# megaease/easevoice-trainer

Measured on AMD Instinct MI355X. Metric: audio-seconds/sec trained (s2), higher is better.
Workload: dtype bf16; 1 GPU; s2 SoVITS generator+discriminator GAN step, batch=16/GPU, 4 s 32 kHz clips (T=200 frames), configs/s2.json, random-init weights; global_batch=16, parallelism=dp1, launch=hip-graph replay (3 graphs/step)

## Files before the change

easevoice_trainer_amd/csrc/elementwise.hip:

```cpp
#include "evt_common.h"
#include "../../include/evt.h"

namespace {

__device__ __forceinline__ void store_w(void* base, long idx, float w, int dtype) {
  if (dtype == EVT_DT_HALF) reinterpret_cast<h16_t*>(base)[idx] = f2h(w);
  else reinterpret_cast<float*>(base)[idx] = w;
}

__device__ __forceinline__ long reg_idx(const evt_wlayout& L, int d0, int d1, int kk) {
  const int chunk = d1 / L.reg_ck, cc = d1 - chunk * L.reg_ck;
  return (((long)d0 * L.reg_nchunk + chunk) * L.reg_kp + kk) * L.reg_ck + cc;
}

__device__ __forceinline__ long alt_idx(const evt_wlayout& L, int d0, int d1, int kk) {
  const int chunk = d0 / L.alt_ck, cc = d0 - chunk * L.alt_ck;
  if (L.stride == 1) {
    const int t = L.k - 1 - kk;
    return (((long)d1 * L.alt_nchunk + chunk) * L.alt_kp + t) * L.alt_ck + cc;
  }
  const int J = (L.k + L.stride - 1) / L.stride;
  const int ph = kk % L.stride, j = kk / L.stride;
  const int jp = J - 1 - j;
  return ((((long)ph * L.d1 + d1) * L.alt_nchunk + chunk) * L.alt_kp + jp) * L.alt_ck + cc;
// ... 483 lines not shown
  if (found) {
    *scale = *scale * backoff;
    *tracker = 0;
  } else {
    const int ok = *tracker + 1;
    if (ok == interval) {
      const float ns = *scale * growth;
      if (isfinite(ns)) *scale = ns;
      *tracker = 0;
    } else {
      *tracker = ok;
    }
  }
}

__global__ __launch_bounds__(256) void sumsq_kernel(const float* x, long n, float* out) {
  __shared__ float red[4];
  float acc = 0.f;
  for (long i = blockIdx.x * 256L + threadIdx.x; i < n; i += (long)gridDim.x * 256) acc += x[i] * x[i];
  acc = block_reduce_sum_256(acc, red);
  if (threadIdx.x == 0) atomicAdd(out, acc);
}

inline int grid_for(long n, int cap = 8192) {
  long b = (n + 255) / 256;
  if (b > cap) b = cap;
  if (b < 1) b = 1;
  return (int)b;
}

}

#include <stdarg.h>
#include <stdio.h>
static bool g_tags_on = false;
static thread_local char g_last_tag[128] = "";
extern "C" void evt_set_last_tag(const char* fmt, ...) {
  if (!g_tags_on) return;
  va_list ap;
  va_start(ap, fmt);
  vsnprintf(g_last_tag, sizeof(g_last_tag), fmt, ap);
  va_end(ap);
}

extern "C" {

// ... 3 lines not shown
#ifndef EVT_SRC_HASH
#define EVT_SRC_HASH "unknown"
#endif
const char* evt_version(void) { return "evt-hip 0.3 (gfx950, half = " EVT_HALF_NAME ") src=" EVT_SRC_HASH; }
int32_t evt_half_dtype(void) { return EVT_DT_HALF; }

int evt_wn_fold_multi(const evt_wprep_item* items, const int32_t* row_index, int32_t nrows, void* stream) {
  if (!items || !row_index || nrows <= 0) return EVT_EINVAL;
  const int nblocks = ((nrows + 255) / 256) * 256;
  hipLaunchKernelGGL(wn_fold_kernel, dim3(nblocks), dim3(256), 0, (hipStream_t)stream, items, row_index, nrows);
  return evt_check_launch();
}

int evt_wn_fold_groups(const evt_wprep_item* items, const int32_t* group_index, int32_t ngroups, void* stream) {
  if (!items || !group_index || ngroups <= 0) return EVT_EINVAL;
  const int nblocks = ((ngroups + 31) / 32) * 32;
  hipLaunchKernelGGL(wn_fold8_kernel, dim3(nblocks), dim3(256), 0, (hipStream_t)stream, items, group_index, ngroups);
  return evt_check_launch();
}

int evt_wn_grad_multi(const evt_wprep_item* items, const int32_t* row_index, int32_t nrows, void* stream) {
  if (!items || !row_index || nrows <= 0) return EVT_EINVAL;
  hipLaunchKernelGGL(wn_grad_kernel, dim3(nrows), dim3(256), 0, (hipStream_t)stream, items, row_index);
  return evt_check_launch();
}

int evt_add3_scale(int32_t dtype, const void* a, const void* b, const void* c, float scale, void* out, int64_t n,
                   void* stream) {
  if (!a || !out || n <= 0) return EVT_EINVAL;
  hipStream_t st = (hipStream_t)stream;
  if (dtype == EVT_DT_HALF)
    hipLaunchKernelGGL(add3_scale_kernel<h16_t>, dim3(grid_for(n)), dim3(256), 0, st, (const h16_t*)a,
                       (const h16_t*)b, (const h16_t*)c, scale, (h16_t*)out, (long)n);
  else if (dtype == EVT_DT_F32)
    hipLaunchKernelGGL(add3_scale_kernel<float>, dim3(grid_for(n)), dim3(256), 0, st, (const float*)a, (const float*)b,
                       (const float*)c, scale, (float*)out, (long)n);
  else return EVT_EINVAL;
  return evt_check_launch();
}

int evt_leaky_relu(int32_t dtype, const void* x, float slope, void* out, int64_t n, void* stream) {
  if (!x || !out || n <= 0) return EVT_EINVAL;
  if (((uintptr_t)x | (uintptr_t)out) & 15) return EVT_EINVAL;
  hipStream_t st = (hipStream_t)stream;
  if (dtype == EVT_DT_HALF)
    hipLaunchKernelGGL(lrelu_kernel<h16_t>, dim3(grid_for((n + 7) / 8)), dim3(256), 0, st, (const h16_t*)x, slope,
// ... 178 lines not shown
```

easevoice_trainer_amd/hip/conv.py:

```python
import ctypes as C
import os
import math

import torch
from torch import nn

from . import lib as L


class ConvSlot:

    __slots__ = ("module", "layout", "reg", "alt", "dw", "bank", "_pcache", "packed_member", "parts", "dw_extra",
                 "db_part", "used", "wg_used", "wg_dirty", "_wgp")

    def __init__(self, module, layout, bank):
        self.module, self.layout, self.bank = module, layout, bank
        self.reg = self.alt = self.dw = None
        self._pcache = {}
        self.packed_member = False
        self.parts, self.dw_extra, self.db_part, self.used, self.wg_used, self._wgp = 1, None, None, None, 0, None
        self.wg_dirty = False

    def params(self, nseq, lin, in_slope, out_act, out_slope):
        key = (nseq, lin, in_slope, out_act, out_slope, self.bank.impl)
# ... 192 lines not shown
            it.dg = g.grad.data_ptr() if g is not None else None
            it.lay = s.layout
            it.dtype = self.dt
            it.src_d1 = int(getattr(m, "src_d1", 0))
            if self.parts_on and not s.packed_member:
                it.dw_extra = s.dw_extra.data_ptr() if s.parts > 1 else None
                it.dw_part_stride = (s.layout.reg_elems + 127) // 128 * 128
                it.used = s.used.data_ptr()
                bias = getattr(m, "bias", None)
                if bias is not None and not m.transposed:
                    if bias.grad is None:
                        bias.grad = torch.zeros_like(bias)
                    it.db_part, it.db = s.db_part.data_ptr(), bias.grad.data_ptr()
            items.append(it)
            self._group_of_row[len(rows)] = len(groups)
            rows.extend((i, r) for r in range(s.layout.d0))
            groups.extend((i, r, min(8, s.layout.d0 - r)) for r in range(0, s.layout.d0, 8))
        self._group_of_row[len(rows)] = len(groups)
        self._items = L.struct_to_device(items, self.device)
        self._rows = torch.tensor(rows, dtype=torch.int32, device=self.device).contiguous()
        self._groups = torch.tensor(groups, dtype=torch.int32, device=self.device).contiguous()
        self._nrows = len(rows)
        self._grad_stamp = self._grad_ptrs()

    def _grad_ptrs(self):
        out = []
        for s in self.slots:
            m = s.module
            g = m.weight_g if m.weight_norm else None
            b = getattr(m, "bias", None)
            out.append((m.v.grad.data_ptr() if m.v.grad is not None else 0,
                        g.grad.data_ptr() if (g is not None and g.grad is not None) else 0,
                        b.grad.data_ptr() if (b is not None and b.grad is not None) else 0))
        return out

    def fold(self, lo=None, hi=None):
        if self._items is None:
            self.build_tables()
        lo = 0 if lo is None else lo
        hi = self._nrows if hi is None else hi
        if hi <= lo:
            return
        glo, ghi = self._group_of_row.get(lo), self._group_of_row.get(hi)
        if glo is not None and ghi is not None and os.environ.get("EVT_FOLD_GROUPS", "1") != "0":
            grp = C.c_void_p(self._groups.data_ptr() + 12 * glo)
            L.check(L.lib().evt_wn_fold_groups(L.ptr(self._items), grp, ghi - glo, L.stream_ptr()), "evt_wn_fold_groups")
        else:
            rows = C.c_void_p(self._rows.data_ptr() + 8 * lo)
            L.check(L.lib().evt_wn_fold_multi(L.ptr(self._items), rows, hi - lo, L.stream_ptr()), "evt_wn_fold_multi")
        self._repack_frags(lo, hi)

    def frag(self, slot, which):
        key = (id(slot), which)
        f = self._frags.get(key)
        if f is None:
            lay = slot.layout
            if which == "reg":
                rows, ktot, src, elems = lay.d0, lay.reg_nchunk * lay.reg_kp * lay.reg_ck, slot.reg, lay.reg_elems
            else:
                rows, ktot, src, elems = lay.d1, lay.alt_nchunk * lay.alt_kp * lay.alt_ck, slot.alt, lay.alt_elems
            if elems != rows * ktot or rows % 16 or ktot % 32 or not L.is_half(self.dtype):
                raise L.EvtError(f"no fragment-order form for this image ({which}, {rows} x {ktot}, {self.dtype})")
            if self._items is None:
                self.build_tables()
            f = torch.empty(elems, dtype=self.dtype, device=self.device)
            it = L.FragItem()
            it.src, it.dst, it.rows, it.ktot = src.data_ptr(), f.data_ptr(), rows, ktot
            self._frags[key] = f
            self._frag_items.append(it)
            self._frag_rows.append(self._slot_rows[self.slots.index(slot)])
            self._frag_retired.extend(t for t, _n in self._frag_tables.values() if t is not None)
            self._frag_tables.clear()
            one = L.struct_to_device([it], self.device)
# ... 715 lines not shown
```

easevoice_trainer_amd/hip/lib.py:

```python
import ctypes as C
import os

import torch

_HERE = os.path.dirname(os.path.abspath(__file__))
LIB_PATH = os.path.join(os.path.dirname(_HERE), "libevt_hip.so")
LIB_PATH_F16 = os.path.join(os.path.dirname(_HERE), "libevt_hip_f16.so")

DT_F32, DT_BF16, DT_F16 = 0, 1, 2
HALF_DTYPES = (torch.bfloat16, torch.float16)
ACT_NONE, ACT_LRELU, ACT_TANH = 0, 1, 2
IMPL_AUTO, IMPL_NAIVE, IMPL_IGEMM = 0, 1, 2


class EvtError(RuntimeError):
    pass


class ConvParams(C.Structure):
    _fields_ = [
        ("dtype", C.c_int32), ("nseq", C.c_int32), ("lin", C.c_int32), ("cin", C.c_int32), ("cout", C.c_int32),
        ("k", C.c_int32), ("stride", C.c_int32), ("pad", C.c_int32), ("dil", C.c_int32), ("groups", C.c_int32),
        ("transposed", C.c_int32), ("in_slope", C.c_float), ("out_act", C.c_int32), ("out_slope", C.c_float),
        ("impl", C.c_int32),
# ... 37 lines not shown

class FragItem(C.Structure):
    _fields_ = [("src", C.c_void_p), ("dst", C.c_void_p), ("rows", C.c_int32), ("ktot", C.c_int32)]


class WgradParts(C.Structure):
    _fields_ = [("dw_extra", C.c_void_p), ("part_stride", C.c_int64), ("db_part", C.c_void_p), ("used_dev", C.c_void_p),
                ("parts", C.c_int32), ("prev_used", C.c_int32), ("used", C.c_int32), ("dirty0", C.c_int32),
                ("ws", C.c_void_p), ("ws_floats", C.c_int64)]


class Seg(C.Structure):
    _fields_ = [("a", C.c_void_p), ("b", C.c_void_p), ("da", C.c_void_p), ("n", C.c_int64),
                ("scale", C.c_float), ("pad_", C.c_int32)]


class KlParams(C.Structure):
    _fields_ = [("B", C.c_int32), ("T", C.c_int32), ("C", C.c_int32), ("time_inner", C.c_int32),
                ("dt_z_p", C.c_int32), ("dt_logs_q", C.c_int32), ("dt_m_p", C.c_int32), ("dt_logs_p", C.c_int32)]


class AdamWSeg(C.Structure):
    _fields_ = [("begin", C.c_int64), ("end", C.c_int64), ("lr", C.c_float), ("weight_decay", C.c_float)]


class AttnParams(C.Structure):
    _fields_ = [
        ("dtype", C.c_int32), ("B", C.c_int32), ("L", C.c_int32), ("H", C.c_int32), ("D", C.c_int32),
        ("x_len", C.c_int32),
        ("q_stride_b", C.c_int64), ("q_stride_l", C.c_int64), ("q_stride_h", C.c_int64),
        ("o_stride_b", C.c_int64), ("o_stride_l", C.c_int64), ("o_stride_h", C.c_int64),
        ("dropout_p", C.c_float), ("seed", C.c_uint32),
    ]


class SampleParams(C.Structure):
    _fields_ = [("V", C.c_int32), ("eos", C.c_int32), ("top_k", C.c_int32), ("no_eos_steps", C.c_int32),
                ("ymax", C.c_int32), ("top_p", C.c_float), ("temperature", C.c_float),
                ("repetition_penalty", C.c_float), ("seed", C.c_uint32), ("noise_rows", C.c_int32)]


class RowSample(C.Structure):
    _fields_ = [("top_k", C.c_int32), ("top_p", C.c_float), ("temperature", C.c_float),
                ("repetition_penalty", C.c_float)]


# ... 59 lines not shown


def lib():
    _lib = _libs.get(_half)
    if _lib is None:
        path = LIB_PATH if _half == torch.bfloat16 else LIB_PATH_F16
        if not os.path.exists(path):
            raise EvtError(
                f"{path} not found: build it with `python -m easevoice_trainer_amd.build` "
                "(or __graft_entry__.build()). There is no fallback path.")
        _lib = C.CDLL(path)
        _lib.evt_version.restype = C.c_char_p
        _check_fresh(_lib, path)
        _lib.evt_half_dtype.restype = C.c_int32
        if _lib.evt_half_dtype() != (DT_BF16 if _half == torch.bfloat16 else DT_F16):
            raise EvtError(f"{path} serves half code {_lib.evt_half_dtype()}: not the {_half} build")
        _libs[_half] = _lib
        _lib.evt_conv1d_lout.restype = C.c_int32
        _lib.evt_mel_workspace_floats.restype = C.c_int64
        _lib.evt_workspace_bytes.restype = C.c_int64
        _lib.evt_last_kernel_tag.restype = C.c_char_p
        _lib.evt_resunit_bwd_ws_floats.restype = C.c_int64
        _lib.evt_debug_kernel_tags.restype = None
    return _lib


def check(rc: int, what: str) -> None:
    if rc != 0:
        raise EvtError(f"{what} failed with code {rc}")


def dt_of(t: torch.Tensor) -> int:
    return dt_code(t.dtype)


def torch_dtype(dt: int) -> torch.dtype:
    return {DT_F32: torch.float32, DT_BF16: torch.bfloat16, DT_F16: torch.float16}[dt]


def ptr(t):
    if t is None:
        return C.c_void_p(0)
    if not t.is_contiguous():
        raise EvtError("non-contiguous tensor passed to the C ABI")
    return C.c_void_p(t.data_ptr())

# ... 67 lines not shown
```

easevoice_trainer_amd/runtime.py:

```python
import ctypes as C

import torch
from torch import nn

from .hip import lib as L
from .hip.conv import WeightBank

_ALIGN = 64


class ParamArena:

    def __init__(self, model: nn.Module, device, reserve=None):
        self.device = torch.device(device)
        params = [(n, p) for n, p in model.named_parameters()]
        order = [n for n, _ in params]
        for mod_name, mod in model.named_modules():
            fn = getattr(mod, "arena_adjacent", None)
            if fn is None:
                continue
            for group in fn():
                full = [f"{mod_name}.{r}" if mod_name else r for r in group]
                if any(n not in order for n in full):
                    continue
                first = min(order.index(n) for n in full)
                pos = sum(1 for n in order[:first] if n not in full)
                rest = [n for n in order if n not in full]
                order = rest[:pos] + full + rest[pos:]
        by_name = dict(params)
        params = [(n, by_name[n]) for n in order]
        offs, total = {}, 0
# ... 61 lines not shown
        self._table = None
        self._table_lrs = None

    @property
    def param_groups(self):
        return self.groups

    def _segments(self):
        lrs = tuple(g["lr"] for g in self.groups)
        if self._table is None or lrs != self._table_lrs:
            segs = []
            for g in self.groups:
                for b, e in g["ranges"]:
                    segs.append(L.AdamWSeg(b, e, g["lr"], self.weight_decay))
            if len(segs) > 64:
                raise L.EvtError(f"{len(segs)} AdamW segments (max 64): register parameters group-contiguously")
            new = L.struct_to_device(segs, self.arena.device)
            if self._table is None:
                self._table = new
            else:
                self._table.copy_(new)
            self._nseg = len(segs)
            self._table_lrs = lrs
        return self._table, self._nseg

    def step(self, grad_scale=1.0, skip=None):
        self.step_count += 1
        tab, nseg = self._segments()
        a = self.arena
        a.updates += 1
        if skip is not None:
            self._guarded = True
            L.check(L.lib().evt_adamw_flat_dev_guarded(L.ptr(a.param), L.ptr(a.grad), L.ptr(self.exp_avg),
                                                       L.ptr(self.exp_avg_sq), C.c_int64(a.numel), L.ptr(tab), nseg,
                                                       C.c_float(self.betas[0]), C.c_float(self.betas[1]), C.c_float(self.eps),
                                                       L.ptr(self._step_dev), C.c_float(grad_scale), L.ptr(skip),
                                                       L.stream_ptr()), "evt_adamw_flat_dev_guarded")
            return
        L.check(L.lib().evt_adamw_flat_dev(L.ptr(a.param), L.ptr(a.grad), L.ptr(self.exp_avg), L.ptr(self.exp_avg_sq),
                                           C.c_int64(a.numel), L.ptr(tab), nseg, C.c_float(self.betas[0]),
                                           C.c_float(self.betas[1]), C.c_float(self.eps), L.ptr(self._step_dev),
                                           C.c_float(grad_scale), L.stream_ptr()), "evt_adamw_flat_dev")

    def sync_step_count(self):
        if getattr(self, "_guarded", False):
            self.step_count = int(self._step_dev.item())
        return self.step_count
# ... 129 lines not shown
            book.wait_stream(bank._side)
        with torch.cuda.stream(book):
            for lo, hi in grad_rows:
                bank.grads(lo, hi, join=False)
            n = 0
            for lo, hi in ranges:
                if hi > lo:
                    optim.step_range(lo, hi, first and n == 0, grad_scale)
                    n += 1
            for lo, hi in fold_rows:
                bank.fold(lo, hi)

    def book_join(self, all_folded=True):
        if self._book is not None:
            torch.cuda.current_stream(self.device).wait_stream(self._book)
        self.bank.join_side()
        if all_folded:
            self.mark_folded()

    def mark_folded(self):
        a = self.arena
        self._fold_stamp = (a.updates, a.param._version, sum(p._version for p in self.model.parameters()))

    def grad_sumsq(self):
        self._sumsq.zero_()
        L.check(L.lib().evt_sumsq(L.ptr(self.arena.grad), C.c_int64(self.arena.numel), L.ptr(self._sumsq),
                                  L.stream_ptr()), "evt_sumsq")
        return self._sumsq


class DeviceGradScaler:

    def __init__(self, device, init_scale=2.0 ** 16, growth_factor=2.0, backoff_factor=0.5, growth_interval=2000,
                 enabled=True):
        self.device = torch.device(device)
        self.enabled = enabled
        self.growth_factor, self.backoff_factor, self.growth_interval = growth_factor, backoff_factor, growth_interval
        self._scale = torch.full((1,), float(init_scale), dtype=torch.float32, device=self.device)
        self._tracker = torch.zeros(1, dtype=torch.int32, device=self.device)
        self._found = {}
        self._flag_table = None

    def found_inf(self, owner):
        f = self._found.get(id(owner))
        if f is None:
            f = self._found[id(owner)] = torch.zeros(1, dtype=torch.float32, device=self.device)
# ... 40 lines not shown
```

easevoice_trainer_amd/train/s2_engine.py:

```python
import os
from dataclasses import dataclass, field
from types import SimpleNamespace
from typing import Optional

import torch
from torch.nn import functional as F

from ..hip import lib as L
from ..hip.enc import bump_rng
from ..module import commons
from ..module.losses import (discriminator_loss, discriminator_loss_batched, feature_loss, generator_loss, kl_loss,
                             l1_mean_scaled)
from ..module.mel_processing import mel_spectrogram_torch, spec_to_mel_slices
from ..module.models import MultiPeriodDiscriminator, SynthesizerTrn
from ..runtime import DeviceGradScaler, FlatAdamW, ModelRuntime


@dataclass
class S2Losses:
    disc: torch.Tensor
    gen: torch.Tensor
    fm: torch.Tensor
    mel: torch.Tensor
    kl: torch.Tensor
# ... 3 lines not shown
    grad_sumsq_g: Optional[torch.Tensor] = None
    extras: dict = field(default_factory=dict)


class S2Engine:
    def __init__(self, hps: dict, device="cuda:0", dtype=torch.bfloat16, impl=L.IMPL_AUTO, reducer=None, scaler_args=None):
        self.hps, self.device, self.dtype = hps, torch.device(device), dtype
        L.set_half(dtype)
        self.scaler = DeviceGradScaler(self.device, enabled=dtype == torch.float16, **(scaler_args or {}))
        d, m, t = hps["data"], hps["model"], hps["train"]
        self.net_g = SynthesizerTrn(d["filter_length"] // 2 + 1, t["segment_size"] // d["hop_length"],
                                    n_speakers=d["n_speakers"], **m)
        self.net_d = MultiPeriodDiscriminator(m["use_spectral_norm"])
        self.rt_g = ModelRuntime(self.net_g, dtype, self.device, impl)
        self.rt_d = ModelRuntime(self.net_d, dtype, self.device, impl)
        self.reducer = reducer
        self.optim_g = self.optim_d = None
        self.graphs_enabled = False
        self.overlap = (reducer is not None and reducer.active and os.environ.get("EVT_DP_OVERLAP", "1") != "0")
        self.cut_only = (not self.overlap and os.environ.get("EVT_DP_CUT", "0") == "1")
        self.pipe = ((reducer is None or not reducer.active) and self.device.type == "cuda" and not self.cut_only
                     and not self.scaler.enabled
                     and os.environ.get("EVT_BOOK_PIPE", "0") == "1")
        self.dp_d_pieces = max(1, int(os.environ.get("EVT_DP_D_PIECES", "6")))
        self.dp_g_pieces = min(3, max(1, int(os.environ.get("EVT_DP_G_PIECES", "1"))))
        if self.overlap or self.pipe or self.cut_only:
            self.net_g.split_backward = self.pipe or self.dp_g_pieces > 1
            nd = len(self.net_d.discriminators)
            self._d_ranges = [self.rt_d.arena.range_of_prefix(f"discriminators.{i}.") for i in range(nd)]
            self._d_convs = [[m for m in d.modules() if hasattr(m, "_slot")] for d in self.net_d.discriminators]
            self._dec_convs = [m for n, m in self.net_g.dec.named_modules() if hasattr(m, "_slot")]
            self._dec_range = self.rt_g.arena.range_of_prefix("dec.", stop_before="dec.cond.")
            self._fq_convs = [m for sub in (self.net_g.flow, self.net_g.enc_q) for m in sub.modules() if hasattr(m, "_slot")]
            flo, fhi = self.rt_g.arena.range_of_prefix("flow.")
            qlo, qhi = self.rt_g.arena.range_of_prefix("enc_q.")
            if fhi != qlo and qhi != flo:
                raise L.EvtError("data-parallel overlap: flow and enc_q are expected to be adjacent in the gradient arena")
            self._fq_range = (min(flo, qlo), max(fhi, qhi))
            self._d_rows = [self.rt_d.bank.rows_of(c) for c in self._d_convs]
            self._dec_rows = self.rt_g.bank.rows_of(self._dec_convs)
            self._dec_rows_fold = self.rt_g.bank.rows_of([m for m in self._dec_convs if m is not self.net_g.dec.cond])
            self._fq_rows = self.rt_g.bank.rows_of(self._fq_convs)
            early = [(self._dec_range, self.rt_g), (self._fq_range, self.rt_g)] + [(r, self.rt_d) for r in self._d_ranges]
            for (lo, hi), rt in early:
                for p_, view in rt._free:
                    off = (view.data_ptr() - rt.arena.grad.data_ptr()) // 4
# ... 52 lines not shown
            st.y_mel = spec_to_mel_slices(st.spec, st.ids_slice, seg // hop, d["filter_length"], d["n_mel_channels"],
                                          d["sampling_rate"], d["mel_fmin"], d["mel_fmax"])
            st.y_hat_mel = mel_spectrogram_torch(st.y_hat.squeeze(1), d["filter_length"], d["n_mel_channels"],
                                                 d["sampling_rate"], hop, d["win_length"], d["mel_fmin"], d["mel_fmax"])
        st.y_seg = commons.slice_segments_1d(st.y.squeeze(1), st.ids_slice * hop, seg)
        rt_d.bank.weight_grads = True
        if self.device.type == "cuda":
            outs = net_d.forward_batched(st.y_seg, st.y_hat.detach())
            if not backward:
                st.d_losses = [discriminator_loss_batched([o]) for o in outs]
            else:
                st.loss_disc = discriminator_loss_batched(outs)
        else:
            y_d_hat_r, y_d_hat_g, _, _ = net_d(st.y_seg, st.y_hat.detach())
            if not backward:
                st.d_losses = [discriminator_loss([r], [g]) for r, g in zip(y_d_hat_r, y_d_hat_g)]
            else:
                st.loss_disc = discriminator_loss(y_d_hat_r, y_d_hat_g)
        if not backward:
            st.d_done = []
            st.loss_disc = torch.stack([l.detach() for l in st.d_losses]).sum()
            return
        self.scaler.scale(st.loss_disc).backward()
        rt_d.finish_grads()
        if lane is not None:
            main.wait_stream(lane)
            st.y_mel.record_stream(main)
            st.y_hat_mel.record_stream(main)

    def _phase_b(self, st, backward=True):
        t = self.hps["train"]
        net_d, rt_g, rt_d = self.net_d, self.rt_g, self.rt_d
        self.scaler.unscale_(rt_d)
        st.gss_d = rt_d.grad_sumsq() * (st.inv_world * st.inv_world)
        if st.hook_after_d is not None:
            st.hook_after_d()
        if st.do_opt and not getattr(st, "piped", False):
            self.optim_d.step(grad_scale=st.inv_world, **self._skip(rt_d))
            rt_d.prepare()
        rt_d.bank.weight_grads = False
        st.loss_gen, st.loss_fm, st.y_d_hat_g = net_d.generator_losses(st.y_seg, st.y_hat)
        z, z_p, m_p, logs_p, m_q, logs_q = st.lat
        if self.device.type == "cuda" and st.y_mel.dtype == st.y_hat_mel.dtype:
            st.loss_mel = l1_mean_scaled(st.y_hat_mel, st.y_mel, t["c_mel"])
        else:
            st.loss_mel = F.l1_loss(st.y_mel, st.y_hat_mel) * t["c_mel"]
        st.loss_kl = kl_loss(z_p, logs_q, m_p, logs_p, st.z_mask, lens=st.spec_lengths) * t["c_kl"]
        st.loss_gen_all = st.loss_gen + st.loss_fm + st.loss_mel + st.kl_ssl * 1 + st.loss_kl
        if not backward:
            return
        self.scaler.scale(st.loss_gen_all).backward()
        rt_d.bank.weight_grads = True
        rt_g.finish_grads()

    def _skip(self, rt):
        return dict(skip=self.scaler.found_inf(rt)) if self.scaler.enabled else {}

    def _phase_c(self, st):
        self.scaler.unscale_(self.rt_g)
        st.gss_g = self.rt_g.grad_sumsq() * (st.inv_world * st.inv_world)
        if st.do_opt:
            self.optim_g.step(grad_scale=st.inv_world, **self._skip(self.rt_g))
            self.scaler.update()

    @staticmethod
    def _result(st) -> S2Losses:
        z, z_p, m_p, logs_p, m_q, logs_q = st.lat
        return S2Losses(st.loss_disc.detach(), st.loss_gen.detach(), st.loss_fm.detach(), st.loss_mel.detach(),
                        st.loss_kl.detach(), st.kl_ssl.detach(), st.loss_gen_all.detach(), st.gss_d, st.gss_g,
                        extras=dict(y_hat=st.y_hat.detach(), y_hat_mel=st.y_hat_mel.detach(), y_mel=st.y_mel.detach(),
                                    ids_slice=st.ids_slice, z=z.detach(), z_p=z_p.detach(), m_p=m_p.detach(),
                                    logs_p=logs_p.detach(), m_q=m_q.detach(), logs_q=logs_q.detach(),
                                    d_logits=[o.detach() for o in st.y_d_hat_g], quantized=st.q.detach()))

    def _reduce(self, arena):
        if self.reducer is not None:
            self.reducer.all_reduce(arena.grad)

    def _phase_a0(self, st):
        self._phase_a(st, backward=False)

# ... 209 lines not shown
            if ent["seen"] <= self._graph_warmup or captured >= self._graph_max or not self._room_for_capture():
                self.graph_steps["eager"] += 1
                self.graphs_enabled = False
                try:
                    return self.step(*inputs)
                finally:
                    self.graphs_enabled = True
            counts = (self.optim_d.step_count, self.optim_g.step_count)
            try:
                self._capture(ent, inputs)
            except Exception as e:
                import warnings

                warnings.warn(f"HIP-graph capture of the s2 step failed ({e!r}); continuing with eager launches")
                self.optim_d.step_count, self.optim_g.step_count = counts
                torch.cuda.synchronize()
                self.graphs_enabled = False
                return self.step(*inputs)
        for dst, src in zip(ent["static"], inputs):
            if dst is not None:
                dst.copy_(src, non_blocking=True)
        self.optim_d._segments()
        self.optim_g._segments()
        if self.pipe:
            self.rt_g.prepare()
            self.rt_d.prepare()
        for g, after in zip(ent["graphs"], ent["after"]):
            g.replay()
            if after is not None:
                after()
        self.optim_d.note_replayed_step()
        self.optim_g.note_replayed_step()
        if self.pipe:
            self.rt_g.mark_folded()
            self.rt_d.mark_folded()
        self.graph_steps["replayed"] += 1
        return ent["result"]

    def _capture(self, ent, inputs):
        static = [t.clone() if t is not None else None for t in inputs]
        ssl, spec, spec_lengths, y, text, text_lengths, eps, ids_slice = static
        st = SimpleNamespace(ssl=ssl, spec=spec, spec_lengths=spec_lengths, y=y, text=text, text_lengths=text_lengths,
                             eps=eps, ids_slice_in=ids_slice, do_opt=True, hook_after_d=None,
                             inv_world=1.0 / self.reducer.world if self.reducer is not None else 1.0)
        self.optim_d._segments()
        self.optim_g._segments()
        torch.cuda.synchronize()
        pool = torch.cuda.graph_pool_handle()
        graphs, afters = [], []
        for phase, after in self._program():
            g = torch.cuda.CUDAGraph()
            with torch.cuda.graph(g, pool=pool, capture_error_mode="relaxed"):
                phase(st)
            graphs.append(g)
            afters.append(after)
        self.optim_d.step_count -= 1
# ... 3 lines not shown
```

include/evt.h:

```cpp
#ifndef EVT_H
#define EVT_H
#include <stddef.h>
#include <stdint.h>

#ifdef __cplusplus
extern "C" {
#endif
#pragma GCC visibility push(default)

#define EVT_DT_F32 0
#define EVT_DT_BF16 1
#define EVT_DT_F16 2
#define EVT_ACT_NONE 0
#define EVT_ACT_LRELU 1
#define EVT_ACT_TANH 2
#define EVT_IMPL_AUTO 0
#define EVT_IMPL_NAIVE 1
#define EVT_IMPL_IGEMM 2

const char* evt_version(void);
int32_t evt_half_dtype(void);
void evt_debug_kernel_tags(int32_t enable);
const char* evt_last_kernel_tag(void);

// ... 168 lines not shown
} evt_kl_params;
int evt_masked_kl_fwd(const evt_kl_params* p, const void* z_p, const void* logs_q, const void* m_p, const void* logs_p,
                      const int32_t* lens, float* out2, void* stream);
int evt_masked_kl_bwd(const evt_kl_params* p, const void* z_p, const void* logs_q, const void* m_p, const void* logs_p,
                      const int32_t* lens, const float* dloss, const float* count, void* dz_p, void* dlogs_q, void* dm_p,
                      void* dlogs_p, void* stream);

typedef struct evt_adamw_seg { int64_t begin, end; float lr; float weight_decay; } evt_adamw_seg;
int evt_adamw_flat(float* param, const float* grad, float* exp_avg, float* exp_avg_sq, int64_t n,
                   const evt_adamw_seg* segs, int32_t nseg, float beta1, float beta2, float eps, int32_t step,
                   float grad_scale, void* stream);
int evt_adamw_flat_dev(float* param, const float* grad, float* exp_avg, float* exp_avg_sq, int64_t n,
                       const evt_adamw_seg* segs, int32_t nseg, float beta1, float beta2, float eps,
                       int32_t* step_counter, float grad_scale, void* stream);
int evt_adamw_flat_dev_range(float* param, const float* grad, float* exp_avg, float* exp_avg_sq, int64_t lo, int64_t hi,
                             const evt_adamw_seg* segs, int32_t nseg, float beta1, float beta2, float eps,
                             int32_t* step_counter, int32_t bump, float grad_scale, void* stream);
int evt_mpd_fold(int32_t src0_dtype, const void* src0, int32_t n0, int32_t src1_dtype, const void* src1, int32_t n1, int32_t T,
                 const int32_t* periods, int32_t nper, void* const* outs, int32_t out_dtype, void* stream);
int evt_mpd_unfold(int32_t grad_dtype, const void* const* douts, const int32_t* periods, int32_t nper, int32_t b0, int32_t n,
                   int32_t T, int32_t dsrc_dtype, void* dsrc, void* stream);

int evt_sumsq(const float* x, int64_t n, float* out, void* stream);

int evt_scaler_unscale(float* grad, int64_t n, const float* scale, float* found_inf, void* stream);
int evt_adamw_flat_dev_guarded(float* param, const float* grad, float* exp_avg, float* exp_avg_sq, int64_t n,
                               const evt_adamw_seg* segs, int32_t nseg, float beta1, float beta2, float eps,
                               int32_t* step_counter, float grad_scale, const float* skip, void* stream);
int evt_scaler_update(float* scale, int32_t* growth_tracker, float* const* found_inf, int32_t nflags, float growth_factor,
                      float backoff_factor, int32_t growth_interval, void* stream);

typedef struct evt_gemm_params {
  int32_t dtype;
  int32_t M, N, K;
  int32_t relu;
} evt_gemm_params;
int evt_gemm_bf16_layout(const evt_gemm_params* g, evt_wlayout* out);
int evt_gemm_bf16_fwd(const evt_gemm_params* g, const void* x, const void* w_reg, const void* w_alt, const float* bias,
                      void* y, void* stream);
int evt_gemm_bf16_bwd_data(const evt_gemm_params* g, const void* dy, const void* w_reg, const void* w_alt, void* dx,
                           void* stream);
int evt_gemm_bf16_bwd_weight(const evt_gemm_params* g, const void* x, const void* dy, float* dw, float* dbias,
                             void* stream);

typedef struct evt_gemm_epilogue {
  float dropout_p;
// ... 183 lines not shown
```

Before: 3442 audio-s/s.

## Fuse weight-norm grad, AdamW update, grad sumsq and weight repack into one kernel

Adds a wn_step8 kernel that, per group of 8 output rows, computes the weight-norm gradient from dW, applies AdamW to v and g in place, accumulates grad sum-of-squares partials, and repacks the new normalized weights into reg/alt bf16 layouts. The remaining parameters go through range-based AdamW and sumsq kernels that skip the fused holes, replacing the separate finish_grads, sumsq, optimizer step and prepare/fold passes for both D and G. The goal is fewer passes over the parameter, grad and optimizer-state memory and fewer launches inside the graphs. In exchange it adds complex planning code, and because it is enabled by default it changes the numerics order slightly.

```diff
diff --git a/easevoice_trainer_amd/csrc/elementwise.hip b/easevoice_trainer_amd/csrc/elementwise.hip
--- a/easevoice_trainer_amd/csrc/elementwise.hip
+++ b/easevoice_trainer_amd/csrc/elementwise.hip
@@ -529,6 +529,288 @@
   if (threadIdx.x == 0) atomicAdd(out, acc);
 }
 
+struct AdamConst { float b1, b2, eps, bc1, bc2_sqrt, gscale; };
+constexpr int WS_U = 4;
+
+__device__ __forceinline__ float adamw_elem(float p, float g, float* m, float* v, float lr, float wd, const AdamConst& c) {
+#pragma clang fp contract(off)
+  const float gr = g * c.gscale;
+  const float pv = p * __builtin_fmaf(-lr, wd, 1.f);
+  const float mv = c.b1 * *m + (1.f - c.b1) * gr;
+  const float vv = c.b2 * *v + (1.f - c.b2) * gr * gr;
+  *m = mv; *v = vv;
+  const float denom = sqrtf(vv) / c.bc2_sqrt + c.eps;
+  return pv - (lr / c.bc1) * (mv / denom);
+}
+
+__device__ __forceinline__ int adamw_seg_of(const evt_adamw_seg* segs, int nseg, long i) {
+  for (int s = 0; s < nseg; ++s)
+    if (i >= segs[s].begin && i < segs[s].end) return s;
+  return -1;
+}
+
+struct WnStepArgs {
+  float* param; float* m; float* v2;
+  const evt_adamw_seg* segs; int nseg;
+  float b1, b2, eps, gscale;
+  const int* stepp; const float* skip;
+  float* partials;
+};
+
+__device__ __forceinline__ void wn_step_row(const evt_wprep_item& it, int d0, const WnStepArgs& a, const AdamConst& c,
+                                            int si_v, int si_g, float& sq, float* red, float* gnew_s, float* scale_out) {
+#pragma clang fp contract(off)
+  const evt_wlayout& L = it.lay;
+  const int n = (it.src_d1 ? it.src_d1 : L.d1) * L.k;
+  const long vo = (it.v - a.param) + (long)d0 * n;
+  float* v = a.param + vo;
+  float* m = a.m + vo;
+  float* v2 = a.v2 + vo;
+  float* dv = it.dv + (long)d0 * n;
+  if (it.used) {
+    const int nu = it.used[0], nb = it.used[1];
+    if (nu > 1 && it.dw_extra) {
+      const int row_floats = L.reg_nchunk * L.reg_kp * L.reg_ck;
+      const long ro = (long)d0 * row_floats;
+      fold_slabs_row(const_cast<float*>(it.dw) + ro, it.dw_extra + ro, it.dw_part_stride, nu, row_floats);
+    }
+    if (nb > 0 && it.db_part && it.db && threadIdx.x == 0) {
+      float s = 0.f;
+      for (int k = 0; k < nb; ++k) s += it.db_part[(long)k * L.d0 + d0];
+      it.db[d0] = 0.f + s;
+    }
+  }
+  const bool upd = si_v >= 0;
+  const float lr = upd ? a.segs[si_v].lr : 0.f, wd = upd ? a.segs[si_v].weight_decay : 0.f;
+  if (!it.g) {
+    for (int e = threadIdx.x; e < n; e += 256) {
+      const int d1 = e / L.k, kk = e - d1 * L.k;
+      const float gv = 0.f + it.dw[reg_idx(L, d0, d1, kk)];
+      dv[e] = gv;
+      sq = __builtin_fmaf(gv, gv, sq);
+      if (upd) {
+        float mv = m[e], vv = v2[e];
+        v[e] = adamw_elem(v[e], gv, &mv, &vv, lr, wd, c);
+        m[e] = mv; v2[e] = vv;
+      }
+    }
+    if (threadIdx.x == 0) *scale_out = 1.f;
+    return;
+  }
+  float ss = 0.f, dot = 0.f;
+  for (int e0 = threadIdx.x; e0 < n; e0 += 256 * WS_U) {
+    float x[WS_U], w[WS_U];
+#pragma unroll
+    for (int u = 0; u < WS_U; ++u) {
+      const int e = e0 + 256 * u;
+      if (e < n) {
+        const int d1 = e / L.k, kk = e - d1 * L.k;
+        x[u] = v[e];
+        w[u] = it.dw[reg_idx(L, d0, d1, kk)];
+      }
+    }
+#pragma unroll
+    for (int u = 0; u < WS_U; ++u)
+      if (e0 + 256 * u < n) {
+        ss = __builtin_fmaf(x[u], x[u], ss);
+        dot = __builtin_fmaf(x[u], w[u], dot);
+      }
+  }
+  ss = block_reduce_sum_256(ss, red);
+  dot = block_reduce_sum_256(dot, red);
+  const float norm = sqrtf(ss);
+  const float gval = it.g[d0];
+  if (threadIdx.x == 0) {
+    const float dgv = 0.f + dot / norm;
+    it.dg[d0] = dgv;
+    sq = __builtin_fmaf(dgv, dgv, sq);
+    float gn = gval;
+    if (si_g >= 0) {
+      const long go = (it.g - a.param) + d0;
+      float mv = a.m[go], vv = a.v2[go];
+      gn = adamw_elem(gval, dgv, &mv, &vv, a.segs[si_g].lr, a.segs[si_g].weight_decay, c);
+      a.m[go] = mv; a.v2[go] = vv;
+      a.param[go] = gn;
+    }
+    *gnew_s = gn;
+  }
+  const float s1 = gval / norm, s2 = dot / ss;
+  float ssn = 0.f;
+  for (int e0 = threadIdx.x; e0 < n; e0 += 256 * WS_U) {
+    float x[WS_U], w[WS_U], mv[WS_U], vv[WS_U];
+#pragma unroll
+    for (int u = 0; u < WS_U; ++u) {
+      const int e = e0 + 256 * u;
+      if (e < n) {
+        const int d1 = e / L.k, kk = e - d1 * L.k;
+        x[u] = v[e];
+        w[u] = it.dw[reg_idx(L, d0, d1, kk)];
+        if (upd) { mv[u] = m[e]; vv[u] = v2[e]; }
+      }
+    }
+#pragma unroll
+    for (int u = 0; u < WS_U; ++u) {
+      const int e = e0 + 256 * u;
+      if (e < n) {
+        const float gv = __builtin_fmaf(s1, __builtin_fmaf(-s2, x[u], w[u]), 0.f);
+        dv[e] = gv;
+        sq = __builtin_fmaf(gv, gv, sq);
+        float xn = x[u];
+        if (upd) {
+          xn = adamw_elem(xn, gv, &mv[u], &vv[u], lr, wd, c);
+          m[e] = mv[u]; v2[e] = vv[u];
+          v[e] = xn;
+        }
+        ssn = __builtin_fmaf(xn, xn, ssn);
+      }
+    }
+  }
+  ssn = block_reduce_sum_256(ssn, red);
+  if (threadIdx.x == 0) *scale_out = *gnew_s / sqrtf(ssn);
+}
+
+__global__ __launch_bounds__(256) void wn_step8_kernel(const evt_wprep_item* items, const int32_t* groups, int ngroups,
+                                                       WnStepArgs a) {
+  __shared__ float red[4];
+  __shared__ float gnew_s;
+  __shared__ float scale_s[8];
+  __shared__ __attribute__((aligned(16))) h16_t src_s[8][F8_ROW];
+  if (a.skip && *a.skip != 0.f) return;
+  const int grp = fold_group_of_block(blockIdx.x, ngroups);
+  if (grp < 0) return;
+  const evt_wprep_item it = items[groups[3 * grp]];
+  const int d0 = groups[3 * grp + 1], nr = groups[3 * grp + 2];
+  const evt_wlayout& L = it.lay;
+  const int d1n = it.src_d1 ? it.src_d1 : L.d1;
+  const int n = d1n * L.k;
+  const int tid = threadIdx.x;
+  AdamConst c;
+  {
+    const float stepf = (float)*a.stepp;
+    c.b1 = a.b1; c.b2 = a.b2; c.eps = a.eps; c.gscale = a.gscale;
+    c.bc1 = 1.f - powf(a.b1, stepf);
+    c.bc2_sqrt = sqrtf(1.f - powf(a.b2, stepf));
+  }
+  const int si_v = adamw_seg_of(a.segs, a.nseg, (it.v - a.param) + (long)d0 * n);
+  const int si_g = it.g ? adamw_seg_of(a.segs, a.nseg, (it.g - a.param) + d0) : -1;
+  float sq = 0.f;
+  for (int r = 0; r < nr; ++r) wn_step_row(it, d0 + r, a, c, si_v, si_g, sq, red, &gnew_s, &scale_s[r]);
+  sq = block_reduce_sum_256(sq, red);
+  if (tid == 0) a.partials[grp] = sq;
+  float* vb = a.param + (it.v - a.param);
+  const bool fast = nr == 8 && it.dtype == EVT_DT_HALF && it.reg && it.alt && (d0 & 7) == 0 && (L.alt_ck & 7) == 0 &&
+                    (n & 3) == 0 && L.reg_kp <= F8_KMAX && L.k <= F8_KMAX && L.reg_ck * L.k <= F8_ROW &&
+                    (L.reg_ck & 7) == 0 && (L.d1 % L.reg_ck) == 0 && ((L.reg_ck * L.k) & 3) == 0;
+  if (!fast) {
+    for (int r = 0; r < nr; ++r) {
+      const float scale = scale_s[r];
+      const float* v = vb + (long)(d0 + r) * n;
+      for (int e = tid; e < n; e += 256) {
+        const int d1 = e / L.k, kk = e - d1 * L.k;
+        const float w = v[e] * scale;
+        if (it.reg) store_w(it.reg, reg_idx(L, d0 + r, d1, kk), w, it.dtype);
+        if (it.alt) store_w(it.alt, alt_idx(L, d0 + r, d1, kk), w, it.dtype);
+      }
+    }
+    return;
+  }
+  const int k = L.k, kp = L.reg_kp, ck = L.reg_ck;
+  h16_t* regp = reinterpret_cast<h16_t*>(it.reg);
+  h16_t* altp = reinterpret_cast<h16_t*>(it.alt);
+  const long reg_row = (long)L.reg_nchunk * kp * ck;
+  const int seg_max = (F8_ROW / (ck * k)) * ck;
+  for (int c0 = 0; c0 < L.d1; c0 += seg_max) {
+    const int seg = min(seg_max, L.d1 - c0);
+    const int src_cols = max(0, min(seg, d1n - c0));
+    const int segk = src_cols * k;
+    const int f4_per_row = segk >> 2;
+    for (int q = tid; q < 8 * f4_per_row; q += 256) {
+      const int r = q / f4_per_row, f = q - r * f4_per_row;
+      const f32x4 x = *reinterpret_cast<const f32x4*>(vb + (long)(d0 + r) * n + (long)c0 * k + 4 * f);
+      const float sc = scale_s[r];
+      h16_t w[4];
+#pragma unroll
+      for (int u = 0; u < 4; ++u) w[u] = f2h(x[u] * sc);
+      *reinterpret_cast<uint2*>(&src_s[r][4 * f]) = *reinterpret_cast<uint2*>(w);
+    }
+    __syncthreads();
+    {
+      const int pieces = seg * kp / 8;
+      const int ck8 = ck >> 3;
+      for (int q = tid; q < 8 * pieces; q += 256) {
+        const int r = q / pieces, pc = q - r * pieces;
+        const int cc8 = pc % ck8, t2 = pc / ck8;
+        const int kk = t2 % kp, chl = t2 / kp;
+        const int dl0 = chl * ck + cc8 * 8;
+        h16_t w[8];
+#pragma unroll
+        for (int j = 0; j < 8; ++j) w[j] = (kk < k && dl0 + j < src_cols) ? src_s[r][(dl0 + j) * k + kk] : (h16_t)0;
+        *reinterpret_cast<uint4*>(regp + (long)(d0 + r) * reg_row + (long)(c0 / ck) * kp * ck + pc * 8) =
+            *reinterpret_cast<uint4*>(w);
+      }
+    }
+    for (int q = tid; q < segk; q += 256) {
+      const int dl = q / k, kk = q - dl * k;
+      h16_t w[8];
+#pragma unroll
+      for (int j = 0; j < 8; ++j) w[j] = src_s[j][q];
+      *reinterpret_cast<uint4*>(altp + alt_idx(L, d0, c0 + dl, kk)) = *reinterpret_cast<uint4*>(w);
+    }
+    __syncthreads();
+  }
+}
+
+__device__ __forceinline__ int range_of_tile(const evt_adamw_range* rg, int nrange, long t) {
+  int lo = 0, hi = nrange - 1;
+  while (lo < hi) {
+    const int mid = (lo + hi + 1) >> 1;
+    if (rg[mid].tile0 <= t) lo = mid; else hi = mid - 1;
+  }
+  return lo;
+}
+
+__global__ __launch_bounds__(256) void adamw_ranges_kernel(float* p, const float* g, float* m, float* v,
+                                                           const evt_adamw_range* rg, int nrange, long ntiles, float b1,
+                                                           float b2, float eps, const int* stepp, float gscale,
+                                                           const float* skip) {
+  if (skip && *skip != 0.f) return;
+  AdamConst c;
+  const float stepf = (float)*stepp;
+  c.b1 = b1; c.b2 = b2; c.eps = eps; c.gscale = gscale;
+  c.bc1 = 1.f - powf(b1, stepf);
+  c.bc2_sqrt = sqrtf(1.f - powf(b2, stepf));
+  for (long t = blockIdx.x; t < ntiles; t += gridDim.x) {
+    const evt_adamw_range r = rg[range_of_tile(rg, nrange, t)];
+    const long i = r.begin + (t - r.tile0) * 256 + threadIdx.x;
+    if (i < r.end) {
+      float mv = m[i], vv = v[i];
+      p[i] = adamw_elem(p[i], g[i], &mv, &vv, r.lr, r.weight_decay, c);
+      m[i] = mv; v[i] = vv;
+    }
+  }
+}
+
+__global__ __launch_bounds__(256) void sumsq_ranges_kernel(const float* x, const evt_adamw_range* rg, int nrange, long ntiles,
+                                                           float* partials) {
+  __shared__ float red[4];
+  float acc = 0.f;
+  for (long t = blockIdx.x; t < ntiles; t += gridDim.x) {
+    const evt_adamw_range r = rg[range_of_tile(rg, nrange, t)];
+    const long i = r.begin + (t - r.tile0) * 256 + threadIdx.x;
+    if (i < r.end) acc += x[i] * x[i];
+  }
+  acc = block_reduce_sum_256(acc, red);
+  if (threadIdx.x == 0) partials[blockIdx.x] = acc;
+}
+
+__global__ __launch_bounds__(256) void sum_partials_kernel(const float* partials, int n, float* out) {
+  __shared__ float red[4];
+  float acc = 0.f;
+  for (int i = threadIdx.x; i < n; i += 256) acc += partials[i];
+  acc = block_reduce_sum_256(acc, red);
+  if (threadIdx.x == 0) *out = acc;
+}
+
 inline int grid_for(long n, int cap = 8192) {
   long b = (n + 255) / 256;
   if (b > cap) b = cap;
@@ -578,6 +860,48 @@
 int evt_wn_grad_multi(const evt_wprep_item* items, const int32_t* row_index, int32_t nrows, void* stream) {
   if (!items || !row_index || nrows <= 0) return EVT_EINVAL;
   hipLaunchKernelGGL(wn_grad_kernel, dim3(nrows), dim3(256), 0, (hipStream_t)stream, items, row_index);
+  return evt_check_launch();
+}
+
+int evt_wn_step_groups(const evt_wprep_item* items, const int32_t* group_index, int32_t ngroups, float* param,
+                       float* exp_avg, float* exp_avg_sq, const evt_adamw_seg* segs, int32_t nseg, float beta1, float beta2,
+                       float eps, int32_t* step_counter, int32_t bump, float grad_scale, const float* skip,
+                       float* group_sumsq, void* stream) {
+  if (!items || !group_index || ngroups <= 0 || !param || !exp_avg || !exp_avg_sq || !segs || nseg <= 0 || nseg > 64 ||
+      !step_counter || !group_sumsq)
+    return EVT_EINVAL;
+  if (bump) hipLaunchKernelGGL(counter_inc_kernel, dim3(1), dim3(1), 0, (hipStream_t)stream, step_counter, skip);
+  WnStepArgs a{param, exp_avg, exp_avg_sq, segs, nseg, beta1, beta2, eps, grad_scale, (const int*)step_counter, skip,
+               group_sumsq};
+  const int nblocks = ((ngroups + 31) / 32) * 32;
+  hipLaunchKernelGGL(wn_step8_kernel, dim3(nblocks), dim3(256), 0, (hipStream_t)stream, items, group_index, ngroups, a);
+  return evt_check_launch();
+}
+
+int evt_adamw_flat_dev_ranges(float* param, const float* grad, float* exp_avg, float* exp_avg_sq,
+                              const evt_adamw_range* ranges, int32_t nranges, int64_t ntiles, float beta1, float beta2,
+                              float eps, int32_t* step_counter, int32_t bump, float grad_scale, const float* skip,
+                              void* stream) {
+  if (!param || !grad || !exp_avg || !exp_avg_sq || !ranges || nranges <= 0 || ntiles <= 0 || !step_counter)
+    return EVT_EINVAL;
+  if (bump) hipLaunchKernelGGL(counter_inc_kernel, dim3(1), dim3(1), 0, (hipStream_t)stream, step_counter, skip);
+  const int blocks = (int)(ntiles < 8192 ? ntiles : 8192);
+  hipLaunchKernelGGL(adamw_ranges_kernel, dim3(blocks), dim3(256), 0, (hipStream_t)stream, param, grad, exp_avg, exp_avg_sq,
+                     ranges, nranges, (long)ntiles, beta1, beta2, eps, (const int*)step_counter, grad_scale, skip);
+  return evt_check_launch();
+}
+
+int evt_sumsq_ranges(const float* x, const evt_adamw_range* ranges, int32_t nranges, int64_t ntiles, float* partials,
+                     int32_t nblocks, void* stream) {
+  if (!x || !ranges || nranges <= 0 || ntiles <= 0 || !partials || nblocks <= 0 || nblocks > 65535) return EVT_EINVAL;
+  hipLaunchKernelGGL(sumsq_ranges_kernel, dim3(nblocks), dim3(256), 0, (hipStream_t)stream, x, ranges, nranges,
+                     (long)ntiles, partials);
+  return evt_check_launch();
+}
+
+int evt_sum_partials(const float* partials, int32_t n, float* out, void* stream) {
+  if (!partials || n <= 0 || !out) return EVT_EINVAL;
+  hipLaunchKernelGGL(sum_partials_kernel, dim3(1), dim3(256), 0, (hipStream_t)stream, partials, n, out);
   return evt_check_launch();
 }
 
diff --git a/easevoice_trainer_amd/hip/conv.py b/easevoice_trainer_amd/hip/conv.py
--- a/easevoice_trainer_amd/hip/conv.py
+++ b/easevoice_trainer_amd/hip/conv.py
@@ -238,6 +238,7 @@
         self._groups = torch.tensor(groups, dtype=torch.int32, device=self.device).contiguous()
         self._nrows = len(rows)
         self._grad_stamp = self._grad_ptrs()
+        self._step_plan = None
 
     def _grad_ptrs(self):
         out = []
@@ -265,6 +266,80 @@
             rows = C.c_void_p(self._rows.data_ptr() + 8 * lo)
             L.check(L.lib().evt_wn_fold_multi(L.ptr(self._items), rows, hi - lo, L.stream_ptr()), "evt_wn_fold_multi")
         self._repack_frags(lo, hi)
+
+    def plan_step(self, arena):
+        if self._items is None:
+            self.build_tables()
+        p0, g0, n = arena.param.data_ptr(), arena.grad.data_ptr(), arena.numel
+
+        def at(t):
+            if t is None or t.grad is None or not t.is_contiguous() or not t.grad.is_contiguous():
+                return None
+            o = t.data_ptr() - p0
+            if o < 0 or o % 4 or o // 4 + t.numel() > n or t.grad.data_ptr() - g0 != o:
+                return None
+            return o // 4
+
+        groups, at_row, inelig, holes, owned = [], {}, [], [], []
+        for i, s in enumerate(self.slots):
+            m = s.module
+            r0, r1 = self._slot_rows[i]
+            at_row[r0] = len(groups)
+            ok = (not isinstance(m, PackedConv) and not s.packed_member and s.layout.reg_elems > 0
+                  and s.layout.alt_elems > 0)
+            ov = at(m.v) if ok else None
+            og = at(m.weight_g) if (ok and m.weight_norm) else None
+            ok = ok and ov is not None and (og is not None or not m.weight_norm)
+            if ok and m.v.numel() != s.layout.d0 * (int(getattr(m, "src_d1", 0)) or s.layout.d1) * s.layout.k:
+                ok = False
+            owned.append(ok)
+            if not ok:
+                if inelig and inelig[-1][1] == r0:
+                    inelig[-1][1] = r1
+                else:
+                    inelig.append([r0, r1])
+                continue
+            groups.extend((i, r, min(8, s.layout.d0 - r)) for r in range(0, s.layout.d0, 8))
+            holes.append((ov, ov + m.v.numel()))
+            if og is not None:
+                holes.append((og, og + m.weight_g.numel()))
+        at_row[self._nrows] = len(groups)
+        table = torch.tensor(groups or [(0, 0, 0)], dtype=torch.int32, device=self.device).contiguous()
+        self._step_plan = dict(arena=arena, groups=table, ngroups=len(groups), at_row=at_row, owned=owned,
+                               inelig=[tuple(r) for r in inelig], holes=sorted(holes))
+        return self._step_plan
+
+    def step_plan(self, arena):
+        p = self._step_plan
+        if p is None or p["arena"] is not arena:
+            p = self.plan_step(arena)
+        return p
+
+    def step_rows(self, optim, lo=None, hi=None, grad_scale=1.0, skip=None, bump=True, partials=None):
+        plan = self.step_plan(optim.arena)
+        lo = 0 if lo is None else lo
+        hi = self._nrows if hi is None else hi
+        glo, ghi = plan["at_row"].get(lo), plan["at_row"].get(hi)
+        if glo is None or ghi is None:
+            raise L.EvtError("step_rows: the row range must start and end at layer boundaries (rows_of)")
+        ng = ghi - glo
+        if ng <= 0:
+            return 0
+        if partials is None:
+            partials = getattr(self, "_step_partials", None)
+            if partials is None or partials.numel() < plan["ngroups"]:
+                partials = self._step_partials = torch.zeros(plan["ngroups"], dtype=torch.float32, device=self.device)
+        if partials.numel() < ng:
+            raise L.EvtError("step_rows: the partial-sum buffer is smaller than the number of groups")
+        tab, nseg = optim._segments()
+        a = optim.arena
+        grp = C.c_void_p(plan["groups"].data_ptr() + 12 * glo)
+        L.check(L.lib().evt_wn_step_groups(L.ptr(self._items), grp, ng, L.ptr(a.param), L.ptr(optim.exp_avg),
+                                           L.ptr(optim.exp_avg_sq), L.ptr(tab), nseg, optim.betas[0], optim.betas[1],
+                                           optim.eps, L.ptr(optim._step_dev), 1 if bump else 0, grad_scale, L.ptr(skip),
+                                           L.ptr(partials), L.stream_ptr()), "evt_wn_step_groups")
+        self._repack_frags(lo, hi)
+        return ng
 
     def frag(self, slot, which):
         key = (id(slot), which)
diff --git a/easevoice_trainer_amd/hip/lib.py b/easevoice_trainer_amd/hip/lib.py
--- a/easevoice_trainer_amd/hip/lib.py
+++ b/easevoice_trainer_amd/hip/lib.py
@@ -83,6 +83,11 @@
 
 class AdamWSeg(C.Structure):
     _fields_ = [("begin", C.c_int64), ("end", C.c_int64), ("lr", C.c_float), ("weight_decay", C.c_float)]
+
+
+class AdamWRange(C.Structure):
+    _fields_ = [("begin", C.c_int64), ("end", C.c_int64), ("tile0", C.c_int64), ("lr", C.c_float),
+                ("weight_decay", C.c_float)]
 
 
 class AttnParams(C.Structure):
@@ -188,6 +193,15 @@
         _lib.evt_last_kernel_tag.restype = C.c_char_p
         _lib.evt_resunit_bwd_ws_floats.restype = C.c_int64
         _lib.evt_debug_kernel_tags.restype = None
+        vp, i32, i64, f32 = C.c_void_p, C.c_int32, C.c_int64, C.c_float
+        _lib.evt_wn_step_groups.argtypes = [vp, vp, i32, vp, vp, vp, vp, i32, f32, f32, f32, vp, i32, f32, vp, vp, vp]
+        _lib.evt_wn_step_groups.restype = C.c_int
+        _lib.evt_adamw_flat_dev_ranges.argtypes = [vp, vp, vp, vp, vp, i32, i64, f32, f32, f32, vp, i32, f32, vp, vp]
+        _lib.evt_adamw_flat_dev_ranges.restype = C.c_int
+        _lib.evt_sumsq_ranges.argtypes = [vp, vp, i32, i64, vp, i32, vp]
+        _lib.evt_sumsq_ranges.restype = C.c_int
+        _lib.evt_sum_partials.argtypes = [vp, i32, vp, vp]
+        _lib.evt_sum_partials.restype = C.c_int
     return _lib
 
 
diff --git a/easevoice_trainer_amd/runtime.py b/easevoice_trainer_amd/runtime.py
--- a/easevoice_trainer_amd/runtime.py
+++ b/easevoice_trainer_amd/runtime.py
@@ -7,6 +7,44 @@
 from .hip.conv import WeightBank
 
 _ALIGN = 64
+
+
+def subtract_ranges(ranges, holes):
+    out, h = [], 0
+    holes = list(holes)
+    for b, e, *attrs in ranges:
+        at = b
+        while h < len(holes) and holes[h][1] <= at:
+            h += 1
+        j = h
+        while j < len(holes) and holes[j][0] < e:
+            hb, he = holes[j]
+            if hb > at:
+                out.append((at, hb, *attrs))
+            at = max(at, he)
+            j += 1
+        if at < e:
+            out.append((at, e, *attrs))
+    return out
+
+
+def align_holes(holes):
+    out = []
+    for b, e in sorted(holes):
+        e = (e + _ALIGN - 1) // _ALIGN * _ALIGN
+        if out and out[-1][1] >= b:
+            out[-1][1] = max(out[-1][1], e)
+        else:
+            out.append([b, e])
+    return [tuple(r) for r in out]
+
+
+def tile_ranges(ranges, tile=256):
+    out, t = [], 0
+    for b, e, *attrs in ranges:
+        out.append((b, e, t, *attrs))
+        t += (e - b + tile - 1) // tile
+    return out, t
 
 
 class ParamArena:
@@ -114,7 +152,39 @@
                 self._table.copy_(new)
             self._nseg = len(segs)
             self._table_lrs = lrs
+            for rt in getattr(self, "_range_tables", {}).values():
+                if rt["n"]:
+                    rt["table"].copy_(L.struct_to_device(self._range_structs(rt["holes"])[0], self.arena.device))
         return self._table, self._nseg
+
+    def complement_ranges(self, holes):
+        segs = sorted((b, e, g["lr"], self.weight_decay) for g in self.groups for b, e in g["ranges"])
+        return subtract_ranges(segs, align_holes(holes))
+
+    def _range_structs(self, holes):
+        rows, ntiles = tile_ranges(self.complement_ranges(holes))
+        return [L.AdamWRange(b, e, t, lr, wd) for b, e, t, lr, wd in rows], ntiles
+
+    def ranges_table(self, holes):
+        self._segments()
+        key = tuple(holes)
+        tabs = self.__dict__.setdefault("_range_tables", {})
+        rt = tabs.get(key)
+        if rt is None:
+            structs, ntiles = self._range_structs(holes)
+            rt = tabs[key] = dict(holes=list(holes), n=len(structs), ntiles=ntiles,
+                                  table=L.struct_to_device(structs, self.arena.device) if structs else None)
+        return rt
+
+    def step_ranges(self, rt, bump, grad_scale=1.0, skip=None):
+        if not rt["n"]:
+            return
+        a = self.arena
+        L.check(L.lib().evt_adamw_flat_dev_ranges(L.ptr(a.param), L.ptr(a.grad), L.ptr(self.exp_avg),
+                                                  L.ptr(self.exp_avg_sq), L.ptr(rt["table"]), rt["n"], rt["ntiles"],
+                                                  self.betas[0], self.betas[1], self.eps, L.ptr(self._step_dev),
+                                                  1 if bump else 0, grad_scale, L.ptr(skip), L.stream_ptr()),
+                "evt_adamw_flat_dev_ranges")
 
     def step(self, grad_scale=1.0, skip=None):
         self.step_count += 1
@@ -290,6 +360,45 @@
         a = self.arena
         self._fold_stamp = (a.updates, a.param._version, sum(p._version for p in self.model.parameters()))
 
+    def _fused_tables(self, optim):
+        plan = self.bank.step_plan(self.arena)
+        ft = self.__dict__.setdefault("_fused", {}).get(id(optim))
+        if ft is None or ft["plan"] is not plan:
+            holes = plan["holes"]
+            rows, ntiles = tile_ranges(subtract_ranges([(0, self.arena.numel)], align_holes(holes)))
+            structs = [L.AdamWRange(b, e, t, 0.0, 0.0) for b, e, t in rows]
+            nblk = min(ntiles, 512)
+            ft = self._fused[id(optim)] = dict(
+                plan=plan, optim=optim, adam=optim.ranges_table(holes), ss_n=len(structs), ss_tiles=ntiles, ss_blocks=nblk,
+                ss_table=L.struct_to_device(structs, self.device) if structs else None,
+                partials=torch.zeros(max(1, plan["ngroups"] + nblk), dtype=torch.float32, device=self.device))
+        return ft
+
+    def step_fused(self, optim, grad_scale=1.0):
+        bank, a = self.bank, self.arena
+        bank.join_side()
+        bank.check_tables()
+        ft = self._fused_tables(optim)
+        plan = ft["plan"]
+        self.gather_free_grads()
+        for lo, hi in plan["inelig"]:
+            bank.grads(lo, hi, join=False)
+        optim.step_count += 1
+        a.updates += 1
+        ng = bank.step_rows(optim, None, None, grad_scale, None, bump=True, partials=ft["partials"])
+        optim.step_ranges(ft["adam"], bump=ng == 0, grad_scale=grad_scale)
+        n = ng
+        if ft["ss_n"]:
+            L.check(L.lib().evt_sumsq_ranges(L.ptr(a.grad), L.ptr(ft["ss_table"]), ft["ss_n"], ft["ss_tiles"],
+                                             C.c_void_p(ft["partials"].data_ptr() + 4 * ng), ft["ss_blocks"],
+                                             L.stream_ptr()), "evt_sumsq_ranges")
+            n += ft["ss_blocks"]
+        L.check(L.lib().evt_sum_partials(L.ptr(ft["partials"]), n, L.ptr(self._sumsq), L.stream_ptr()), "evt_sum_partials")
+        for lo, hi in plan["inelig"]:
+            bank.fold(lo, hi)
+        self.mark_folded()
+        return self._sumsq
+
     def grad_sumsq(self):
         self._sumsq.zero_()
         L.check(L.lib().evt_sumsq(L.ptr(self.arena.grad), C.c_int64(self.arena.numel), L.ptr(self._sumsq),
diff --git a/easevoice_trainer_amd/train/s2_engine.py b/easevoice_trainer_amd/train/s2_engine.py
--- a/easevoice_trainer_amd/train/s2_engine.py
+++ b/easevoice_trainer_amd/train/s2_engine.py
@@ -49,6 +49,9 @@
         self.pipe = ((reducer is None or not reducer.active) and self.device.type == "cuda" and not self.cut_only
                      and not self.scaler.enabled
                      and os.environ.get("EVT_BOOK_PIPE", "0") == "1")
+        self.fused = ((reducer is None or not reducer.active) and self.device.type == "cuda" and not self.scaler.enabled
+                      and not self.pipe and not self.cut_only and not self.overlap
+                      and os.environ.get("EVT_WN_STEP", "1") != "0")
         self.dp_d_pieces = max(1, int(os.environ.get("EVT_DP_D_PIECES", "6")))
         self.dp_g_pieces = min(3, max(1, int(os.environ.get("EVT_DP_G_PIECES", "1"))))
         if self.overlap or self.pipe or self.cut_only:
@@ -147,7 +150,10 @@
             st.loss_disc = torch.stack([l.detach() for l in st.d_losses]).sum()
             return
         self.scaler.scale(st.loss_disc).backward()
-        rt_d.finish_grads()
+        if self._fused_step(st):
+            rt_d.bank.join_side()
+        else:
+            rt_d.finish_grads()
         if lane is not None:
             main.wait_stream(lane)
             st.y_mel.record_stream(main)
@@ -156,11 +162,15 @@
     def _phase_b(self, st, backward=True):
         t = self.hps["train"]
         net_d, rt_g, rt_d = self.net_d, self.rt_g, self.rt_d
-        self.scaler.unscale_(rt_d)
-        st.gss_d = rt_d.grad_sumsq() * (st.inv_world * st.inv_world)
+        fused = self._fused_step(st)
+        if fused:
+            st.gss_d = rt_d.step_fused(self.optim_d, grad_scale=st.inv_world) * (st.inv_world * st.inv_world)
+        else:
+            self.scaler.unscale_(rt_d)
+            st.gss_d = rt_d.grad_sumsq() * (st.inv_world * st.inv_world)
         if st.hook_after_d is not None:
             st.hook_after_d()
-        if st.do_opt and not getattr(st, "piped", False):
+        if st.do_opt and not getattr(st, "piped", False) and not fused:
             self.optim_d.step(grad_scale=st.inv_world, **self._skip(rt_d))
             rt_d.prepare()
         rt_d.bank.weight_grads = False
@@ -176,12 +186,22 @@
             return
         self.scaler.scale(st.loss_gen_all).backward()
         rt_d.bank.weight_grads = True
-        rt_g.finish_grads()
+        if fused:
+            rt_g.bank.join_side()
+        else:
+            rt_g.finish_grads()
+
+    def _fused_step(self, st):
+        return self.fused and st.do_opt and st.hook_after_d is None and not getattr(st, "piped", False)
 
     def _skip(self, rt):
         return dict(skip=self.scaler.found_inf(rt)) if self.scaler.enabled else {}
 
     def _phase_c(self, st):
+        if self._fused_step(st):
+            st.gss_g = self.rt_g.step_fused(self.optim_g, grad_scale=st.inv_world) * (st.inv_world * st.inv_world)
+            self.scaler.update()
+            return
         self.scaler.unscale_(self.rt_g)
         st.gss_g = self.rt_g.grad_sumsq() * (st.inv_world * st.inv_world)
         if st.do_opt:
@@ -437,7 +457,7 @@
                 dst.copy_(src, non_blocking=True)
         self.optim_d._segments()
         self.optim_g._segments()
-        if self.pipe:
+        if self.pipe or self.fused:
             self.rt_g.prepare()
             self.rt_d.prepare()
         for g, after in zip(ent["graphs"], ent["after"]):
@@ -446,7 +466,7 @@
                 after()
         self.optim_d.note_replayed_step()
         self.optim_g.note_replayed_step()
-        if self.pipe:
+        if self.pipe or self.fused:
             self.rt_g.mark_folded()
             self.rt_d.mark_folded()
         self.graph_steps["replayed"] += 1
diff --git a/include/evt.h b/include/evt.h
--- a/include/evt.h
+++ b/include/evt.h
@@ -214,6 +214,19 @@
                    int32_t T, int32_t dsrc_dtype, void* dsrc, void* stream);
 
 int evt_sumsq(const float* x, int64_t n, float* out, void* stream);
+
+typedef struct evt_adamw_range { int64_t begin, end, tile0; float lr; float weight_decay; } evt_adamw_range;
+int evt_wn_step_groups(const evt_wprep_item* items, const int32_t* group_index, int32_t ngroups, float* param,
+                       float* exp_avg, float* exp_avg_sq, const evt_adamw_seg* segs, int32_t nseg, float beta1, float beta2,
+                       float eps, int32_t* step_counter, int32_t bump, float grad_scale, const float* skip,
+                       float* group_sumsq, void* stream);
+int evt_adamw_flat_dev_ranges(float* param, const float* grad, float* exp_avg, float* exp_avg_sq,
+                              const evt_adamw_range* ranges, int32_t nranges, int64_t ntiles, float beta1, float beta2,
+                              float eps, int32_t* step_counter, int32_t bump, float grad_scale, const float* skip,
+                              void* stream);
+int evt_sumsq_ranges(const float* x, const evt_adamw_range* ranges, int32_t nranges, int64_t ntiles, float* partials,
+                     int32_t nblocks, void* stream);
+int evt_sum_partials(const float* partials, int32_t n, float* out, void* stream);
 
 int evt_scaler_unscale(float* grad, int64_t n, const float* scale, float* found_inf, void* stream);
 int evt_adamw_flat_dev_guarded(float* param, const float* grad, float* exp_avg, float* exp_avg_sq, int64_t n,
```

Result: slower. 3385 audio-s/s (-1.7%).
